# Crocodoctopus/zkstark

Measured on AMD Instinct MI355X. Metric: field-elements/s through LDE+Merkle+FRI (full STARK-101 prover), higher is better.
Workload: dtype u32 (mod 3*2^30+1) + SHA-256

## Files before the change

zkstark_amd/build.py:

```python
import concurrent.futures
import hashlib
import os
import shutil
import subprocess
import sys

HERE = os.path.dirname(os.path.abspath(__file__))
CSRC = os.path.join(HERE, "csrc")
OBJDIR = os.path.join(HERE, "build")
LIB = os.path.join(HERE, "libzkstark_amd.so")
HASHFILE = LIB + ".hash"
SOURCES = ["kernels.hip", "ntt_fast.hip", "domain.hip", "zkstark.hip", "batch.hip", "shard.hip", "verify.hip", "grind.hip", "host_sha.cpp", "version.cpp"]
HEADERS = ["field.hpp", "sha256.hpp", "blake2s.hpp", "sha256_quad.hpp", "fieldhash.hpp", "fieldhash_f64.hpp", "kernels.hpp", "transcript.hpp", "host_sha.hpp", "internal.hpp", "pool.hpp",
           "shard.hpp", "board.hpp", "peer.hpp", os.path.join("..", "..", "include", "zkstark_amd.h")]
ARCH = "gfx950"
FLAGS = ["-O3", "-std=c++17", f"--offload-arch={ARCH}", "-fPIC", "-Wall", "-Wno-unused-function"]
FLAGS += os.environ.get("ZK_BUILD_DEFS", "").split()


def _read(rel):
    with open(os.path.join(CSRC, rel), "rb") as f:
        return f.read()


def source_hash():
    h = hashlib.sha256()
    for rel in SOURCES + HEADERS:
        h.update(os.path.basename(rel).encode() + b"\0")
        h.update(_read(rel))
        h.update(b"\0")
    h.update(" ".join(FLAGS).encode())
    return h.hexdigest()[:24]


def built_hash():
    if not os.path.exists(LIB):
        return None
    try:
        with open(HASHFILE) as f:
            side = f.read().strip()
        if side and os.path.getmtime(HASHFILE) >= os.path.getmtime(LIB):
            return side
    except OSError:
        pass
    try:
        with open(LIB, "rb") as f:
# ... 68 lines not shown
```

zkstark_amd/csrc/internal.hpp:

```cpp
#pragma once
#include <hip/hip_runtime.h>

#include <cstddef>
#include <cstring>
#include <string>
#include <vector>

#include "../../include/zkstark_amd.h"
#include "field.hpp"
#include "kernels.hpp"
#include "transcript.hpp"

struct zk_channel {
    zk::Channel ch;
};

namespace zk {
namespace impl {

int fail(int code, const char* fmt, ...);
const char* last_error();

#define HIPCHK(expr)                                                                          \
    do {                                                                                      \
// ... 8 lines not shown
template <> struct AbiMin<zk_shard_options>   { static constexpr uint32_t v = 48;   static constexpr const char* name = "zk_shard_options"; };
template <> struct AbiMin<zk_shard_stats>     { static constexpr uint32_t v = 112;  static constexpr const char* name = "zk_shard_stats"; };
template <> struct AbiMin<zk_shard_plan_info> { static constexpr uint32_t v = 200;  static constexpr const char* name = "zk_shard_plan_info"; };
template <> struct AbiMin<zk_chain_probe>     { static constexpr uint32_t v = 48;   static constexpr const char* name = "zk_chain_probe"; };
template <class T> inline size_t abi_bytes(const T* p, const char* who) {
    static_assert(sizeof(T) >= AbiMin<T>::v && offsetof(T, struct_size) == 0, "a struct of the C ABI shrank or lost its size field");
    const uint32_t n = p->struct_size;
    if (n < AbiMin<T>::v || n > (1u << 16) || (n > AbiMin<T>::v && n < sizeof(T))) {
        fail(ZK_ERR_INVALID, "%s: %s.struct_size is %u; the caller sets it to sizeof(%s) before the call (ZK_STRUCT_INIT): at least %u bytes "
                             "(ABI version 6), %zu in this library (ABI version %u) -- was the caller compiled against another zkstark_amd.h?",
             who, AbiMin<T>::name, n, AbiMin<T>::name, AbiMin<T>::v, sizeof(T), (unsigned)ZK_ABI_VERSION);
        return 0;
    }
    return n < sizeof(T) ? n : sizeof(T);
}
template <class T> inline int abi_put(T* out, const T& src, const char* who) {
    const size_t k = abi_bytes(out, who);
    if (!k) return ZK_ERR_INVALID;
    memcpy(reinterpret_cast<char*>(out) + sizeof(uint32_t), reinterpret_cast<const char*>(&src) + sizeof(uint32_t), k - sizeof(uint32_t));
    return ZK_OK;
}
template <class T> inline int abi_get(const T* in, T* local, const char* who) {
    const size_t k = abi_bytes(in, who);
    if (!k) return ZK_ERR_INVALID;
    memset(static_cast<void*>(local), 0, sizeof(T));
    memcpy(static_cast<void*>(local), in, k);
    local->struct_size = (uint32_t)sizeof(T);
    return ZK_OK;
}

constexpr uint32_t kMaxQueries = 64;
constexpr uint32_t kHostTopSingle = 8;
constexpr uint32_t kMaxHostLog = 10;
constexpr size_t kMailValsOff = kMailDigests + ((size_t)8 << kMaxHostLog);
constexpr size_t kMailWords = kMailValsOff + ((size_t)2 << kMaxHostLog);
constexpr uint32_t kMaxRadixLog = 8;

inline int check_proof_size(const char* who, uint32_t log_n, uint32_t log_b, uint32_t log_extra = 0) {
    if (log_n < 2 || log_b < 1 || log_b > 5 || log_n + log_b + log_extra > 30)
        return fail(ZK_ERR_INVALID, "%s: need 2 <= log_n, 1 <= log_blowup <= 5, log_n + log_blowup%s <= 30 (got %u, %u)", who,
                    log_extra ? " + log_batch" : "", log_n, log_b);
    if (log_n == 3)
        return fail(ZK_ERR_INVALID, "%s: n = 8 is degenerate for the Fibonacci-square constraints (the degree asserts of prover.rs:156/:169 would fail)", who);
    return ZK_OK;
}

struct Plan {
    uint32_t nd = 0;
    uint32_t bits[kMaxDigits] = {0};
};
Plan make_plan(uint32_t log_m);
uint32_t pick_logC(uint32_t log_total, uint32_t logR);

struct DevTable {
    uint32_t* lo = nullptr;
    uint32_t* hi = nullptr;
    uint32_t lo_bits = 0;
    PowTable view() const { return PowTable{lo, hi, lo_bits}; }
};
int build_table(uint32_t root, uint32_t log_order, DevTable* t);
void free_table(DevTable* t);

int run_dif(const uint32_t* src, uint32_t* data, uint32_t log_m, const Plan& pl, PowTable tw_inv, uint32_t L, uint32_t scale_mont,
            hipStream_t s, Profiler* prof = nullptr, uint32_t batch = 1, size_t src_stride = 0, size_t data_stride = 0);
int run_dit(uint32_t* data, uint32_t log_m, const Plan& pl, PowTable tw, uint32_t L, hipStream_t s);

constexpr uint32_t kGrindHostMaxBits = 10;
struct Grinder;
// ... 59 lines not shown
```

zkstark_amd/csrc/zkstark.hip:

```cpp
#include <hip/hip_runtime.h>

#include <algorithm>
#include <chrono>
#include <cstdarg>
#include <cstdio>
#include <cstdlib>
#include <cstring>
#include <atomic>
#include <condition_variable>
#include <functional>
#include <mutex>
#include <new>
#include <thread>
#include <string>
#include <vector>

#include "../../include/zkstark_amd.h"
#include "field.hpp"
#include "kernels.hpp"
#include "sha256.hpp"
#include "transcript.hpp"
#include "host_sha.hpp"
#include "internal.hpp"
#include "pool.hpp"

using namespace zk;
using namespace zk::impl;

struct zk_ctx {
    int device = 0;
    uint32_t log_n = 0, log_b = 0, L = 0;
    size_t n = 0, N = 0, B = 0;
    uint32_t R = 0;
    hipStream_t stream = nullptr;
    zk_dom* dom = nullptr;
    uint32_t* d_trace = nullptr;
    uint32_t* d_coef = nullptr;
    uint32_t* d_layers = nullptr;
    std::vector<size_t> layer_off, layer_len;
    uint32_t* d_trees = nullptr;
    std::vector<size_t> tree_off;
    uint64_t* d_gather_off = nullptr;
    uint32_t* d_gather_out = nullptr;
    uint64_t* h_gather_off = nullptr;
    uint32_t* h_gather_out = nullptr;
    uint64_t* dm_gather_off = nullptr;
    uint32_t* dm_gather_out = nullptr;
    const uint32_t* host_nodes[40] = {};
    size_t host_node_cnt[40] = {};
    const uint32_t* host_vals[40] = {};
    std::vector<const uint32_t*> fetch_vals, fetch_nodes;
    std::vector<uint32_t> fetch_vdev;
    std::vector<uint64_t> fetch_ditems;
    std::vector<uint8_t> commit_buf;
    bool pending_top = false;
    uint32_t pending_tree = 0;
    size_t open_nv = 0, open_ndg = 0, open_vi = 0;
    bool open_pending = false;
    uint32_t* h_small = nullptr;
    uint32_t* h_mailbox = nullptr;
    uint32_t* d_mailbox = nullptr;
    uint32_t* d_counter = nullptr;
    bool counters_dirty = false;
    uint32_t mail_seq = 0;
    uint32_t tree_seq[40] = {};
    bool early = false, early_ok = false, gate_pending = false;
    uint32_t* h_gate = nullptr;
    uint32_t* d_gate = nullptr;
    uint32_t* h_dyn = nullptr;
    uint32_t* d_dyn = nullptr;
    uint32_t gate_seq = 0;
    uint32_t host_top = 0, host_tail = 0;
    Pool* pool = nullptr;
    uint32_t* h_stage = nullptr;
    uint32_t* d_stage = nullptr;
    size_t stage_words = 0, stage_used = 0;
    ScatterSeg* h_segs = nullptr;
    ScatterSeg* d_segs = nullptr;
    uint32_t n_segs = 0;
    double seg_words = 0;
    std::vector<uint32_t> tail_vals;
    uint32_t tail_log = 0;
    bool tail_have = false;
    double t_wait = 0, t_host_hash = 0, t_launch = 0;
    bool tail = false;
    uint32_t hinv_host = 0;
    uint32_t queries = 1;
    uint32_t grind = 0;
    Grinder* grinder = nullptr;
    uint32_t fold = 1;
    uint64_t skipped_layers = 0, skipped_trees = 0;
    bool coset = false;
    uint8_t tree_steps[40] = {};
    uint32_t stop = 0;
    uint32_t* d_final = nullptr;
    std::vector<uint32_t> final_poly;
    int hash = 0;
    bool checks = false;
    uint32_t* d_check = nullptr;
    DevTable ones;
    size_t gather_cap = 0;
    size_t device_bytes = 0;
    double setup_ms = 0;
    bool have_trace = false, have_lde = false;
    uint32_t first = 0, last = 0;
    zk_transcript_info info{};
    Profiler prof;
    zk_kernel_stat kstat[K_COUNT] = {};
};

namespace {

template <typename T>
int dmalloc(zk_ctx* c, T** p, size_t bytes) {
// ... 75 lines not shown
    if (rc) return rc;
    HIPCHK(launch_compose_merkle(a, c->d_trees + c->tree_off[1], c->stream, prof_of(c), mail_of(c, 1, true), c->hash));
    return ZK_OK;
}
int do_fold_commit(zk_ctx* c, uint32_t round, uint32_t beta_raw) {
    FoldArgs a;
    int rc = fold_args(c->dom, c->d_layers + c->layer_off[1 + round], c->d_layers + c->layer_off[2 + round], c->L - round, round, beta_raw, a);
    if (rc) return rc;
    HIPCHK(launch_fold_merkle(a, c->d_trees + c->tree_off[2 + round], c->stream, prof_of(c), mail_of(c, 2 + round, true), c->hash));
    return ZK_OK;
}

int wait_mail(zk_ctx* c, uint32_t seq) {
    double t0 = now_us();
    int rc = wait_flag(c->h_mailbox, seq, c->stream);
    c->t_wait += now_us() - t0;
    if (rc) c->counters_dirty = true;
    return rc;
}

int read_root(zk_ctx* c, uint32_t tree, uint8_t out[32]) {
    int rc = wait_mail(c, c->tree_seq[tree]);
    if (rc) return rc;
    digest_words_to_bytes(c->h_mailbox + kMailDigests, out);
    return ZK_OK;
}

uint32_t* stage_alloc(zk_ctx* c, size_t words) {
    if (c->stage_used + words > c->stage_words) return nullptr;
    uint32_t* p = c->h_stage + c->stage_used;
    c->stage_used += (words + 7) & ~(size_t)7;
    return p;
}
int stage_seg(zk_ctx* c, const uint32_t* src, size_t dst, size_t words, uint32_t kind) {
    if (c->n_segs >= 4 * 34) return fail(ZK_ERR_STATE, "scatter segment table full");
    c->h_segs[c->n_segs++] = ScatterSeg{(uint64_t)(src - c->h_stage), (uint64_t)dst, (uint32_t)words, kind};
    c->seg_words += (double)words;
    return ZK_OK;
}

int read_commit(zk_ctx* c, uint32_t tree, uint8_t root[32]) {
    const uint32_t H = top_of(c, tree);
    if (!H) return read_root(c, tree, root);
    const size_t cnt = (size_t)1 << H;
    uint32_t* nodes = stage_alloc(c, (2 * cnt - 1) * 8);
    if (!nodes) return fail(ZK_ERR_STATE, "host staging buffer exhausted");
    int rc = wait_mail(c, c->tree_seq[tree]);
    if (rc) return rc;
    double t0 = now_us();
    memcpy(nodes + 8 * (cnt - 1), c->h_mailbox + kMailDigests, cnt * 32);
    const uint32_t sub_log = host_sub_log();
    if (H > sub_log && c->pool) {
        const uint32_t top = H - sub_log;
        c->pool->run((size_t)1 << top, 1, [&](size_t sub) { host_sha_reduce_sub(nodes, H, top, sub); });
        host_sha_reduce(nodes, top);
    } else {
        host_sha_reduce(nodes, H);
    }
    digest_words_to_bytes(nodes, root);
    c->t_host_hash += now_us() - t0;
    if (c->tail_have && c->tail_log == layer_log(c, tree) && tree >= 1) {
        c->tail_vals.assign(c->h_mailbox + kMailValsOff, c->h_mailbox + kMailValsOff + ((size_t)1 << c->tail_log));
    }
    c->host_nodes[tree] = nodes;
    c->host_node_cnt[tree] = 2 * cnt - 1;
    return stage_seg(c, nodes, c->tree_off[tree], (cnt - 1) * 8, 0);
}

int host_fold_commit(zk_ctx* c, uint32_t round, uint32_t beta_raw, uint8_t root[32]) {
    const uint32_t log_out = c->L - round - 1;
    const size_t half = (size_t)1 << log_out;
    const double t_begin = now_us();
    uint32_t* vals = stage_alloc(c, half);
    uint32_t* nodes = stage_alloc(c, (2 * half - 1) * 8);
    if (!vals || !nodes) return fail(ZK_ERR_STATE, "host staging buffer exhausted");
    const zk_dom* d = c->dom;
    const uint32_t cc_m = to_mont(mulmod(beta_raw % P, d->fold_k[round]));
    const uint32_t step_m = to_mont(powmod(c->hinv_host, (uint64_t)1 << round));
    const uint32_t* in = c->tail_vals.data();
    uint32_t xinv_m = to_mont(1);
    for (size_t i = 0; i < half; ++i) {
        uint32_t u = in[i], v = in[i + half];
        vals[i] = add(mont_mul(add(u, v), d->inv2_mont), mont_mul(mont_mul(sub(u, v), xinv_m), cc_m));
        xinv_m = mont_mul(xinv_m, step_m);
    }
    host_sha_leaves(vals, half, nodes + 8 * (half - 1));
    host_sha_reduce(nodes, log_out);
    digest_words_to_bytes(nodes, root);
    c->tail_vals.assign(vals, vals + half);
    c->tail_log = log_out;
    c->t_host_hash += now_us() - t_begin;
    c->tree_steps[2 + round] = 0;
    c->host_vals[2 + round] = vals;
    c->host_nodes[2 + round] = nodes;
    c->host_node_cnt[2 + round] = 2 * half - 1;
    int rc = stage_seg(c, vals, c->layer_off[2 + round], half, 1);
    if (!rc) rc = stage_seg(c, nodes, c->tree_off[2 + round], (2 * half - 1) * 8, 0);
    return rc;
}

int fri_round_commit(zk_ctx* c, uint32_t round, uint32_t beta_raw, uint8_t root[32]) {
    if (c->tail_have && c->tail_log == c->L - round && c->L - round - 1 <= c->host_tail) return host_fold_commit(c, round, beta_raw, root);
    int rc = do_fold_commit(c, round, beta_raw);
    return rc ? rc : read_commit(c, 2 + round, root);
}
bool round_on_host(const zk_ctx* c, uint32_t round) {
    return c->hash == 0 && c->host_top && c->host_tail && c->L >= c->host_tail + 1 && c->L - round <= c->host_tail + 1;
}
bool can_gate(const zk_ctx* c, uint32_t round) { return c->fold == 1 && !c->coset && !c->stop && c->early && c->early_ok && !c->checks && round < c->R && !round_on_host(c, round); }
int enqueue_gated_fold(zk_ctx* c, uint32_t round) {
    FoldArgs a;
    int rc = fold_args(c->dom, c->d_layers + c->layer_off[1 + round], c->d_layers + c->layer_off[2 + round], c->L - round, round, 0u, a);
    if (rc) return rc;
    ++c->gate_seq;
    a.dyn = c->d_dyn + 16 * (c->gate_seq & 1u);
    HIPCHK(hipStreamWaitValue32(c->stream, c->d_gate, c->gate_seq, hipStreamWaitValueEq, 0xFFFFFFFFu));
    c->gate_pending = true;
    HIPCHK(launch_fold_merkle(a, c->d_trees + c->tree_off[2 + round], c->stream, prof_of(c), mail_of(c, 2 + round, true), c->hash));
    return ZK_OK;
}
void release_gate(zk_ctx* c, uint32_t c_mont) {
    c->h_dyn[16 * (c->gate_seq & 1u)] = c_mont;
    __atomic_store_n(c->h_gate, c->gate_seq, __ATOMIC_RELEASE);
    c->gate_pending = false;
}
void release_gated_fold(zk_ctx* c, uint32_t round, uint32_t beta_raw) {
    release_gate(c, to_mont(mulmod(beta_raw % P, c->dom->fold_k[round])));
}
struct GateGuard {
    zk_ctx* c;
    ~GateGuard() { if (c->gate_pending) release_gate(c, 0u); }
};

void begin_proof(zk_ctx* c) {
    c->stage_used = 0; c->n_segs = 0; c->seg_words = 0; c->tail_log = 0; c->tail_have = false;
    c->t_wait = c->t_host_hash = c->t_launch = 0;
    memset(c->host_nodes, 0, sizeof c->host_nodes);
    memset(c->host_node_cnt, 0, sizeof c->host_node_cnt);
    memset(c->host_vals, 0, sizeof c->host_vals);
}
int flush_host_parts(zk_ctx* c) {
    HIPCHK(launch_scatter(c->d_stage, c->d_segs, c->n_segs, c->seg_words, c->d_trees, c->d_layers, c->stream, prof_of(c)));
    c->n_segs = 0;
    c->pending_top = false;
    return ZK_OK;
}
int settle_pending(zk_ctx* c) { return c->pending_top ? flush_host_parts(c) : (int)ZK_OK; }
int last_layer_value(zk_ctx* c, uint32_t* out) {
    const uint32_t* v;
    if (c->tail_have && c->tail_log == c->log_b) v = c->tail_vals.data();
    else {
        HIPCHK(hipMemcpyAsync(c->h_small, c->d_layers + c->layer_off[1 + c->R], c->B * 4, hipMemcpyDeviceToHost, c->stream));
        HIPCHK(hipStreamSynchronize(c->stream));
        v = c->h_small;
    }
    for (size_t i = 1; i < c->B; ++i)
        if (v[i] != v[0]) return fail(ZK_ERR_CHECK, "last FRI layer is not constant (prover.rs:238): trace does not satisfy the constraints");
    *out = v[0];
    return ZK_OK;
}

int final_alloc(zk_ctx* c) {
    return c->d_final ? (int)ZK_OK : dmalloc(c, &c->d_final, (((size_t)1 << kFinalPolyMaxLog) + 1) * 4);
}
int final_poly_value(zk_ctx* c) {
    const uint32_t Rp = c->R - c->stop;
    const size_t cnt = (size_t)1 << c->stop;
    int rc = final_alloc(c);
    if (rc) return rc;
    if ((rc = dom_final_poly(c->dom, c->d_layers + c->layer_off[1 + Rp], c->d_final, c->L - Rp, Rp, (uint32_t)cnt, c->stream, prof_of(c)))) return rc;
    HIPCHK(hipMemcpyAsync(c->h_small, c->d_final, (cnt + 1) * 4, hipMemcpyDeviceToHost, c->stream));
    HIPCHK(hipStreamSynchronize(c->stream));
    if (c->h_small[0])
        return fail(ZK_ERR_CHECK, "final FRI layer has degree >= 2^%u: trace does not satisfy the constraints (%u non-zero coefficients above; cf. prover.rs:238)", c->stop, c->h_small[0]);
    c->final_poly.assign(c->h_small + 1, c->h_small + 1 + cnt);
    return ZK_OK;
}

int do_compose(zk_ctx* c, const uint32_t alpha_raw[3]) {
    return dom_compose(c->dom, c->d_layers + c->layer_off[0], c->d_layers + c->layer_off[1], c->first, c->last,
                       alpha_raw, c->stream, prof_of(c));
}

// ... 4 lines not shown


int checks_alloc(zk_ctx* c) {
    if (c->d_check) return ZK_OK;
    int rc = dmalloc(c, &c->d_check, (c->N + 2) * 4);
    if (rc) return rc;
    return build_table(1, c->log_n, &c->ones);
}
int check_interpolant(zk_ctx* c) {
    const zk_dom* d = c->dom;
    CoefPrepArgs pa{};
    pa.log_n = d->log_n; pa.log_b = d->log_b;
    pa.tw = d->H.view(); pa.wtab = c->ones.view(); pa.ninv_mont = d->ninv_mont;
    pa.nd = d->plan.nd;
    for (uint32_t t = 0; t < d->plan.nd; ++t) pa.dig_bits[t] = d->plan.bits[t];
    HIPCHK(launch_coef_prepare(c->d_coef, c->d_check, pa, c->stream));
    int rc = run_dit(c->d_check, d->log_n, d->plan, d->H.view(), d->L, c->stream);
    if (rc) return rc;
    std::vector<uint32_t> got(c->n), want(c->n);
    HIPCHK(hipMemcpyAsync(got.data(), c->d_check, c->n * 4, hipMemcpyDeviceToHost, c->stream));
    HIPCHK(hipMemcpyAsync(want.data(), c->d_trace, c->n * 4, hipMemcpyDeviceToHost, c->stream));
    HIPCHK(hipStreamSynchronize(c->stream));
    for (size_t i = 0; i + 1 < c->n; ++i)
        if (got[i] != want[i])
            return fail(ZK_ERR_CHECK, "self-check prover.rs:64-66 failed: f(g^%zu) = %u, trace value %u", i, got[i], want[i]);
    return ZK_OK;
}
int check_degree(zk_ctx* c, uint32_t layer, uint32_t want_deg, const char* cite) {
    const uint32_t lg = layer_log(c, layer);
    const size_t m = (size_t)1 << lg;
    const uint32_t* src = c->d_layers + c->layer_off[layer];
    if (lg <= 10) {
        std::vector<uint32_t> v(m);
        if (c->tail_have && c->tail_log == lg && layer >= 2) v.assign(c->tail_vals.begin(), c->tail_vals.begin() + m);
        else {
            HIPCHK(hipMemcpyAsync(v.data(), src, m * 4, hipMemcpyDeviceToHost, c->stream));
            HIPCHK(hipStreamSynchronize(c->stream));
        }
        const uint32_t winv = invmod(root_of_unity(lg));
        for (size_t k = m; k-- > want_deg; ) {
            uint32_t acc = 0, step = powmod(winv, k), x = 1;
            for (size_t i = 0; i < m; ++i) { acc = add(acc, mulmod(v[i], x)); x = mulmod(x, step); }
            if (k > want_deg && acc != 0)
                return fail(ZK_ERR_CHECK, "self-check %s failed: layer %u has a non-zero coefficient of degree %zu > %u", cite, layer, k, want_deg);
            if (k == want_deg && acc == 0)
                return fail(ZK_ERR_CHECK, "self-check %s failed: layer %u has degree below %u", cite, layer, want_deg);
        }
        return ZK_OK;
    }
    const Plan pl = make_plan(lg);
    int rc = run_dif(src, c->d_check, lg, pl, c->dom->Hinv.view(), c->dom->L, 0, c->stream);
    if (rc) return rc;
    uint32_t* res = c->d_check + c->N;
    HIPCHK(hipMemsetAsync(res, 0, 8, c->stream));
    HIPCHK(launch_degree_check(c->d_check, lg, pl.nd, pl.bits, want_deg + 1, res, c->stream));
    uint32_t h[2];
    HIPCHK(hipMemcpyAsync(h, res, 8, hipMemcpyDeviceToHost, c->stream));
    HIPCHK(hipStreamSynchronize(c->stream));
    if (h[0]) return fail(ZK_ERR_CHECK, "self-check %s failed: layer %u has %u non-zero coefficients of degree > %u (a division left a remainder)", cite, layer, h[0], want_deg);
    if (!h[1]) return fail(ZK_ERR_CHECK, "self-check %s failed: layer %u has degree below %u", cite, layer, want_deg);
    return ZK_OK;
}

void open_begin(zk_ctx* c, size_t nvals) {
    c->fetch_vals.assign(nvals, nullptr); c->fetch_vdev.assign(nvals, 0); c->fetch_nodes.clear(); c->fetch_ditems.clear();
    c->open_nv = c->open_ndg = c->open_vi = 0;
}
void open_val(zk_ctx* c, uint32_t layer, size_t x) {
    if (c->host_vals[layer]) c->fetch_vals[c->open_vi++] = c->host_vals[layer] + x;
    else { c->fetch_vdev[c->open_vi++] = (uint32_t)c->open_nv; c->h_gather_off[c->open_nv++] = (uint64_t)c->layer_off[layer] + x; }
}
void open_path(zk_ctx* c, uint32_t tree, size_t m, size_t leaf) {
    for (size_t i = leaf + m - 1; i != 0; i = (i - 1) >> 1) {
        const size_t nd = (i & 1) ? i + 1 : i - 1;
        if (nd < c->host_node_cnt[tree]) c->fetch_nodes.push_back(c->host_nodes[tree] + 8 * nd);
        else { c->fetch_nodes.push_back(c->h_gather_out + 8 * c->open_ndg); ++c->open_ndg; c->fetch_ditems.push_back((uint64_t)c->tree_off[tree] + (uint64_t)nd * 8); }
    }
}
int open_launch(zk_ctx* c) {
    const size_t nv = c->open_nv, ndg = c->open_ndg;
    if (nv + ndg > c->gather_cap) return fail(ZK_ERR_STATE, "gather capacity exceeded");
    if (ndg) memcpy(c->h_gather_off + nv, c->fetch_ditems.data(), ndg * 8);
    for (size_t i = 0; i < c->fetch_vals.size(); ++i)
        if (!c->fetch_vals[i]) c->fetch_vals[i] = c->h_gather_out + 8 * ndg + c->fetch_vdev[i];
    c->open_pending = nv + ndg != 0;
// ... 113 lines not shown
int prove_resident(zk_ctx* c, Channel& ch) {
    if (!c->have_trace) return fail(ZK_ERR_STATE, "zk_prove_resident: no trace uploaded");
    static const bool timing = getenv("ZK_HOST_TIMING") != nullptr;
    HostLaps lap{timing};
    const uint32_t R = c->R;
    ch.data.reserve(ch.data.size() + proof_data_len(c->log_n, c->log_b, c->queries, c->grind, c->fold, c->coset, c->stop));
    c->skipped_layers = c->skipped_trees = 0;
    uint8_t root[32];
    int rc;
    memset(&c->info, 0, sizeof c->info);
    c->info.public_last = c->last;
    c->pending_top = false;
    begin_proof(c);
    GateGuard gate_guard{c};
    if ((rc = do_lde(c))) return rc;
    if (c->checks && ((rc = checks_alloc(c)) || (rc = check_interpolant(c)))) return rc;
    if ((rc = do_merkle(c, 0, true))) return rc;
    if ((rc = read_commit(c, 0, root))) return rc;
    ch.commit_hash(root);
    memcpy(c->info.roots[0], root, 32);
    uint32_t alpha[3];
    for (int i = 0; i < 3; ++i) alpha[i] = c->info.alpha_raw[i] = ch.get_u32();
    if (c->coset) {
        if ((rc = do_compose(c, alpha)) || (rc = do_merkle(c, 1, true, false, fold_steps(R - c->stop, c->fold, 0)))) return rc;
    } else if ((rc = do_compose_commit(c, alpha))) return rc;
    if (can_gate(c, 0) && (rc = enqueue_gated_fold(c, 0))) return rc;
    if ((rc = read_commit(c, 1, root))) return rc;
    if (c->checks && (rc = check_degree(c, 1, (uint32_t)c->n - 1, "prover.rs:148-159/:169 (exact divisions, deg cp = n - 1)"))) return rc;
    ch.commit_hash(root);
    memcpy(c->info.roots[1], root, 32);
    if (c->fold > 1 || c->coset || c->stop) {
        if ((rc = prove_fold_rounds(c, ch))) return rc;
    } else for (uint32_t r = 0; r < R; ++r) {
        uint32_t beta = c->info.beta_raw[r] = ch.get_u32();
        if (c->gate_pending) {
            release_gated_fold(c, r, beta);
            if (can_gate(c, r + 1) && (rc = enqueue_gated_fold(c, r + 1))) return rc;
            if ((rc = read_commit(c, 2 + r, root))) return rc;
        } else if (c->tail_have && c->tail_log == c->L - r && c->L - r - 1 <= c->host_tail) {
            if ((rc = host_fold_commit(c, r, beta, root))) return rc;
        } else {
            if ((rc = do_fold_commit(c, r, beta))) return rc;
            if (can_gate(c, r + 1) && (rc = enqueue_gated_fold(c, r + 1))) return rc;
            if ((rc = read_commit(c, 2 + r, root))) return rc;
        }
        if (c->checks && (rc = check_degree(c, 2 + r, (uint32_t)(c->n >> (r + 1)) - ((c->n >> (r + 1)) ? 1 : 0), "prover.rs:228-251 (FRI layer degree)"))) return rc;
        ch.commit_hash(root);
        memcpy(c->info.roots[2 + r], root, 32);
    }
    lap("lde .. last root");
    if (timing) fprintf(stderr, "[zk timing]   of which: waiting for the device %.1f us, host hashing (tops + tail) %.1f us\n", c->t_wait, c->t_host_hash);
    return prove_finish(c, ch, lap);
}

}

namespace zk {
namespace impl {
int tail_open_begin(zk_ctx* c, size_t x) {
    if (!c || !c->tail) return fail(ZK_ERR_INVALID, "tail_open_begin: not a tail context");
    HIPCHK(hipSetDevice(c->device));
    open_begin(c, 2 * (size_t)c->R);
    for (uint32_t i = 0; i < c->R; ++i) {
        const size_t len = c->N >> i, xi = x % len, nx = (xi + len / 2) % len;
        open_val(c, 1 + i, xi); open_path(c, 1 + i, len, xi);
        open_val(c, 1 + i, nx); open_path(c, 1 + i, len, nx);
    }
    return open_launch(c);
}
int tail_open_end(zk_ctx* c, uint32_t* vals_out, uint8_t* paths_out) {
    int rc = open_wait(c);
    if (rc) return rc;
    for (size_t i = 0; i < c->fetch_vals.size(); ++i) vals_out[i] = *c->fetch_vals[i];
    for (size_t i = 0; i < c->fetch_nodes.size(); ++i) digest_words_to_bytes(c->fetch_nodes[i], paths_out + 32 * i);
    return ZK_OK;
}
int merkle_nodes_to_host(int device, hipStream_t s, const uint32_t* d_heap, size_t first, size_t count, uint8_t* out) {
    if (!count) return ZK_OK;
    HIPCHK(hipSetDevice(device));
    HIPCHK(hipMemcpyAsync(out, d_heap + first * 8, count * 32, hipMemcpyDeviceToHost, s));
    HIPCHK(hipStreamSynchronize(s));
// ... 34 lines not shown
    return mulmod(a % P, invmod(b % P));
}
uint32_t zk_field_rem(uint32_t a, uint32_t rhs) {
    if (rhs == 0) { fail(ZK_ERR_INVALID, "zk_field_rem: remainder by zero (field.rs:89-94 panics)"); return 0; }
    return (a % P) % rhs;
}
uint32_t zk_field_generator(void) {
    static const uint32_t g = [] {
        uint32_t factors[32], nf = 0, p = P - 1;
        for (uint32_t it = 2; p != 1; ++it) {
            if (p % it == 0) factors[nf++] = it;
            while (p % it == 0) p /= it;
        }
        for (uint32_t x = 2; x < P; ++x) {
            bool primitive = true;
            for (uint32_t i = 0; i < nf && primitive; ++i) primitive = powmod(x, (P - 1) / factors[i]) != 1;
            if (primitive) return x;
        }
        return 0u;
    }();
    return g;
}
uint32_t zk_field_order(uint32_t a) {
    a %= P;
    if (a == 0) return 0;
    uint32_t ord = P - 1;
    if (powmod(a, ord / 3) == 1) ord /= 3;
    while (ord % 2 == 0 && powmod(a, ord / 2) == 1) ord /= 2;
    return ord;
}
uint32_t zk_field_root_of_unity(uint32_t log_order) { return log_order > 30 ? 0 : root_of_unity(log_order); }

static int ctx_make(int device, uint32_t log_n, uint32_t log_b, uint32_t shift, bool tail, zk_ctx** out);
static int ctx_team(zk_ctx* c) {
    const uint32_t sub_log = host_sub_log();
    const unsigned want = c->host_top > sub_log ? (1u << (c->host_top - sub_log)) - 1u : 0u;
    if (c->pool && c->pool->workers() == want) return ZK_OK;
    delete c->pool;
    c->pool = nullptr;
    if (!want) return ZK_OK;
    const double spin_us = 5000.0;
    c->pool = new (std::nothrow) Pool(want, spin_us);
    return c->pool ? (int)ZK_OK : fail(ZK_ERR_NOMEM, "out of host memory");
}

int zk_ctx_create(int device, uint32_t log_n, uint32_t log_b, zk_ctx** out) {
    if (!out) return fail(ZK_ERR_INVALID, "zk_ctx_create: out is null");
    *out = nullptr;
    if (int rc = check_proof_size("zk_ctx_create", log_n, log_b)) return rc;
    return ctx_make(device, log_n, log_b, GEN_W, false, out);
}

static int ctx_make(int device, uint32_t log_n, uint32_t log_b, uint32_t shift, bool tail, zk_ctx** out) {
    auto t0 = std::chrono::steady_clock::now();
    HIPCHK(hipSetDevice(device));
    zk_ctx* c = new (std::nothrow) zk_ctx();
    if (!c) return fail(ZK_ERR_NOMEM, "out of host memory");
    c->device = device;
    c->log_n = log_n; c->log_b = log_b; c->L = log_n + log_b;
    c->n = (size_t)1 << log_n; c->B = (size_t)1 << log_b; c->N = c->n << log_b;
    c->R = log_n;
    int rc = ZK_OK;
    auto bail = [&](int code) { zk_ctx_destroy(c); return code; };
#define HIPCHK_C(expr)                                                                        \
    do {                                                                                      \
        hipError_t _e = (expr);                                                               \
        if (_e != hipSuccess) {                                                               \
            zk_ctx_destroy(c);                                                                \
            return fail(ZK_ERR_HIP, "%s failed: %s (%s:%d)", #expr, hipGetErrorString(_e), __FILE__, __LINE__); \
// ... 16 lines not shown
        c->tree_off.push_back(off);
        off += (2 * layer_size(c, l) - 1) * 8;
    }
    size_t tree_words = off;
    if ((rc = dmalloc(c, &c->d_trace, c->n * 4))) return bail(rc);
    if ((rc = dmalloc(c, &c->d_coef, 2 * c->n * 4))) return bail(rc);
    if ((rc = dmalloc(c, &c->d_layers, layer_words * 4))) return bail(rc);
    if ((rc = dmalloc(c, &c->d_trees, tree_words * 4))) return bail(rc);
    c->gather_cap = (size_t)kMaxQueries * (4 + 2 * c->R) * (c->L + 1) + 64;
    if ((rc = dmalloc(c, &c->d_gather_off, c->gather_cap * 8))) return bail(rc);
    if ((rc = dmalloc(c, &c->d_gather_out, c->gather_cap * 32))) return bail(rc);
    HIPCHK_C(hipHostMalloc((void**)&c->h_gather_off, c->gather_cap * 8, hipHostMallocMapped | hipHostMallocCoherent));
    HIPCHK_C(hipHostMalloc((void**)&c->h_gather_out, c->gather_cap * 32, hipHostMallocMapped | hipHostMallocCoherent));
    HIPCHK_C(hipHostGetDevicePointer((void**)&c->dm_gather_off, c->h_gather_off, 0));
    HIPCHK_C(hipHostGetDevicePointer((void**)&c->dm_gather_out, c->h_gather_out, 0));
    HIPCHK_C(hipHostMalloc((void**)&c->h_small, 4096));
    const size_t mail_bytes = kMailWords * 4;
    if ((rc = dmalloc(c, &c->d_counter, 64))) return bail(rc);
    HIPCHK_C(hipMemsetAsync(c->d_counter, 0, 64, c->stream));
    HIPCHK_C(hipHostMalloc((void**)&c->h_mailbox, mail_bytes, hipHostMallocMapped | hipHostMallocCoherent));
    memset(c->h_mailbox, 0, mail_bytes);
    HIPCHK_C(hipHostGetDevicePointer((void**)&c->d_mailbox, c->h_mailbox, 0));
    HIPCHK_C(hipHostMalloc((void**)&c->h_gate, 64, hipHostMallocMapped | hipHostMallocCoherent));
    HIPCHK_C(hipHostMalloc((void**)&c->h_dyn, 2 * 16 * 4, hipHostMallocMapped | hipHostMallocCoherent));
    memset(c->h_gate, 0, 64);
    memset(c->h_dyn, 0, 2 * 16 * 4);
    HIPCHK_C(hipHostGetDevicePointer((void**)&c->d_gate, c->h_gate, 0));
    HIPCHK_C(hipHostGetDevicePointer((void**)&c->d_dyn, c->h_dyn, 0));
    {
        int can = 0;
        if (hipDeviceGetAttribute(&can, hipDeviceAttributeCanUseStreamWaitValue, device) != hipSuccess) { can = 0; (void)hipGetLastError(); }
        c->early_ok = can != 0 && !tail;
    }
    c->stage_words = (size_t)(c->R + 2) * ((size_t)16 << kMaxHostLog) + ((size_t)64 << kMaxHostLog);
    const size_t seg_bytes = 4 * 34 * sizeof(ScatterSeg);
    HIPCHK_C(hipHostMalloc((void**)&c->h_stage, c->stage_words * 4 + seg_bytes, hipHostMallocMapped | hipHostMallocCoherent));
    HIPCHK_C(hipHostGetDevicePointer((void**)&c->d_stage, c->h_stage, 0));
    c->h_segs = reinterpret_cast<ScatterSeg*>(c->h_stage + c->stage_words);
    c->d_segs = reinterpret_cast<ScatterSeg*>(c->d_stage + c->stage_words);
    if (host_sha_available()) {
        c->host_top = 8;
        c->host_tail = 9;
    }
    if (int prc = ctx_team(c)) { zk_ctx_destroy(c); return prc; }
#undef HIPCHK_C
    c->setup_ms = std::chrono::duration<double, std::milli>(std::chrono::steady_clock::now() - t0).count();
    *out = c;
    return ZK_OK;
}

#ifdef ZK_WG_TRACE
extern "C++" { namespace zk { void dump_wg_trace(); } }
#endif

int zk_ctx_destroy(zk_ctx* c) {
    if (!c) return ZK_OK;
    (void)hipSetDevice(c->device);
    if (c->stream) (void)hipStreamSynchronize(c->stream);
#ifdef ZK_WG_TRACE
    zk::dump_wg_trace();
#endif
    dom_free(c->dom);
    if (c->d_trace) (void)hipFree(c->d_trace);
    if (c->d_coef) (void)hipFree(c->d_coef);
    if (c->d_layers) (void)hipFree(c->d_layers);
    if (c->d_trees) (void)hipFree(c->d_trees);
    if (c->d_counter) (void)hipFree(c->d_counter);
    if (c->d_check) (void)hipFree(c->d_check);
// ... 92 lines not shown
    }
    c->stop = stop_log;
    return ZK_OK;
}
uint32_t zk_ctx_get_fri_stop(const zk_ctx* c) { return c ? c->stop : 0; }
int zk_ctx_final_poly(const zk_ctx* c, uint32_t* out, size_t cap, size_t* count) {
    if (!c || !count || (!out && cap)) return fail(ZK_ERR_INVALID, "zk_ctx_final_poly: null argument");
    if (c->final_poly.empty()) return fail(ZK_ERR_STATE, "zk_ctx_final_poly: no proof made yet");
    *count = c->final_poly.size();
    if (c->final_poly.size() > cap) return fail(ZK_ERR_BUFFER, "zk_ctx_final_poly: %zu coefficients, room for %zu", c->final_poly.size(), cap);
    memcpy(out, c->final_poly.data(), c->final_poly.size() * 4);
    return ZK_OK;
}
int zk_ctx_set_queries(zk_ctx* c, uint32_t n_queries) {
    if (!c) return fail(ZK_ERR_INVALID, "null context");
    if (n_queries < 1 || n_queries > kMaxQueries) return fail(ZK_ERR_INVALID, "zk_ctx_set_queries: need 1 <= n_queries <= %u", kMaxQueries);
    c->queries = n_queries;
    return ZK_OK;
}
int zk_ctx_set_grinding(zk_ctx* c, uint32_t grind_bits) {
    if (!c) return fail(ZK_ERR_INVALID, "null context");
    if (c->tail) return fail(ZK_ERR_STATE, "zk_ctx_set_grinding: FRI-tail context");
    if (grind_bits > kMaxGrindBits) return fail(ZK_ERR_INVALID, "zk_ctx_set_grinding: need grind_bits <= %u (got %u)", kMaxGrindBits, grind_bits);
    if (grind_bits > kGrindHostMaxBits && !c->grinder) {
        HIPCHK(hipSetDevice(c->device));
        if (int rc = grinder_create(c->device, c->stream, 1, &c->grinder)) return rc;
    }
    c->grind = grind_bits;
    return ZK_OK;
}

int zk_ctx_set_host_levels(zk_ctx* c, uint32_t top_log, uint32_t tail_log) {
    if (!c) return fail(ZK_ERR_INVALID, "null context");
    if (top_log > kMaxHostLog || tail_log > kMaxHostLog || (tail_log && !top_log))
        return fail(ZK_ERR_INVALID, "zk_ctx_set_host_levels: need top_log, tail_log <= %u, and top_log > 0 when tail_log > 0", kMaxHostLog);
    c->host_top = top_log;
    c->host_tail = tail_log;
    return ctx_team(c);
}
int zk_ctx_get_host_levels(const zk_ctx* c, uint32_t* top_log, uint32_t* tail_log) {
    if (!c || !top_log || !tail_log) return fail(ZK_ERR_INVALID, "zk_ctx_get_host_levels: null argument");
    *top_log = c->host_top;
    *tail_log = c->host_tail;
    return ZK_OK;
}
int zk_ctx_set_checks(zk_ctx* c, int on) {
    if (!c) return fail(ZK_ERR_INVALID, "null context");
    if (c->tail) return fail(ZK_ERR_STATE, "zk_ctx_set_checks: FRI-tail context");
    c->checks = on != 0;
    return ZK_OK;
}
static const char kNoBlake2s[] = "BLAKE2s (hash 2) is not built for this entry point yet";
int zk_ctx_set_hash(zk_ctx* c, int hash_kind) {
    if (!c) return fail(ZK_ERR_INVALID, "null context");
    if (hash_kind != ZK_HASH_SHA256 && hash_kind != ZK_HASH_FIELD && hash_kind != ZK_HASH_BLAKE2S)
        return fail(ZK_ERR_INVALID, "zk_ctx_set_hash: unknown hash %d", hash_kind);
    if (hash_kind == ZK_HASH_BLAKE2S && c->tail) return fail(ZK_ERR_INVALID, "zk_ctx_set_hash: %s", kNoBlake2s);
    c->hash = hash_kind;
    return ZK_OK;
}

int zk_ctx_set_profiling(zk_ctx* c, uint32_t class_mask) {
    if (!c) return fail(ZK_ERR_INVALID, "null context");
    c->prof.mask = class_mask & ((1u << K_COUNT) - 1u);
    return ZK_OK;
}

static int put_kernel_stats(zk_kernel_stat* out, size_t count, const zk_kernel_stat* src, const char* who) {
// ... 894 lines not shown
```

Before: 2.937 billion.

## Parallelize host FRI tail folding and hashing across a thread pool

Moves the host-side FRI tail fold plus SHA-256 leaf/tree hashing into a chunked, pool-parallel routine and allows host tail layers up to 2^13. Tail values are now referenced in place instead of being copied into a vector each round, and scatter segments are split into bounded pieces. The pool size is capped by the usable CPU cores and cgroup quota. Larger host tails require a bigger pinned staging buffer and mailbox, and the parallel path is only used when the tail level is raised.

```diff
diff --git a/zkstark_amd/build.py b/zkstark_amd/build.py
--- a/zkstark_amd/build.py
+++ b/zkstark_amd/build.py
@@ -11,7 +11,7 @@
 LIB = os.path.join(HERE, "libzkstark_amd.so")
 HASHFILE = LIB + ".hash"
 SOURCES = ["kernels.hip", "ntt_fast.hip", "domain.hip", "zkstark.hip", "batch.hip", "shard.hip", "verify.hip", "grind.hip", "host_sha.cpp", "version.cpp"]
-HEADERS = ["field.hpp", "sha256.hpp", "blake2s.hpp", "sha256_quad.hpp", "fieldhash.hpp", "fieldhash_f64.hpp", "kernels.hpp", "transcript.hpp", "host_sha.hpp", "internal.hpp", "pool.hpp",
+HEADERS = ["field.hpp", "sha256.hpp", "blake2s.hpp", "sha256_quad.hpp", "fieldhash.hpp", "fieldhash_f64.hpp", "kernels.hpp", "transcript.hpp", "host_sha.hpp", "host_tail.hpp", "internal.hpp", "pool.hpp",
            "shard.hpp", "board.hpp", "peer.hpp", os.path.join("..", "..", "include", "zkstark_amd.h")]
 ARCH = "gfx950"
 FLAGS = ["-O3", "-std=c++17", f"--offload-arch={ARCH}", "-fPIC", "-Wall", "-Wno-unused-function"]
diff --git a/zkstark_amd/csrc/host_tail.hpp b/zkstark_amd/csrc/host_tail.hpp
--- /dev/null
+++ b/zkstark_amd/csrc/host_tail.hpp
@@ -0,0 +1,74 @@
+#pragma once
+#include <stddef.h>
+#include <stdint.h>
+
+#include "field.hpp"
+#include "host_sha.hpp"
+#include "pool.hpp"
+
+#ifndef ZK_TAIL_CHUNK_LOG
+#define ZK_TAIL_CHUNK_LOG 7
+#endif
+#ifndef ZK_TAIL_TEAM_MIN_LOG
+#define ZK_TAIL_TEAM_MIN_LOG 10
+#endif
+#ifndef ZK_TAIL_TEAM_MAX
+#define ZK_TAIL_TEAM_MAX 7
+#endif
+
+namespace zk {
+
+constexpr uint32_t kTailChunkMinLog = 4;
+constexpr uint32_t kTailChunkLog = ZK_TAIL_CHUNK_LOG;
+constexpr uint32_t kTailTeamMinLog = ZK_TAIL_TEAM_MIN_LOG;
+constexpr uint32_t kTailTeamMax = ZK_TAIL_TEAM_MAX;
+static_assert(kTailChunkLog >= kTailChunkMinLog && kTailChunkLog <= 12, "host tail chunk size");
+static_assert(kTailTeamMinLog > kTailChunkLog && kTailTeamMinLog <= 13, "a team round has at least two chunks");
+static_assert(kTailTeamMax >= 1 && kTailTeamMax <= 15, "host tail team size");
+
+struct HostTailConsts {
+    uint32_t cc_m, step_m;
+};
+inline HostTailConsts host_tail_consts(uint32_t beta_raw, uint32_t fold_k, uint32_t step) {
+    return HostTailConsts{to_mont(mulmod(beta_raw % P, fold_k)), to_mont(step)};
+}
+
+inline void host_tail_fold(const uint32_t* in, size_t half, size_t start, size_t count, uint32_t xinv_m, HostTailConsts k, uint32_t inv2_m,
+                           uint32_t* vals) {
+    for (size_t i = start; i < start + count; ++i) {
+        const uint32_t u = in[i], v = in[i + half];
+        vals[i] = add(mont_mul(add(u, v), inv2_m), mont_mul(mont_mul(sub(u, v), xinv_m), k.cc_m));
+        xinv_m = mont_mul(xinv_m, k.step_m);
+    }
+}
+
+inline void host_tail_round_serial(const uint32_t* in, uint32_t log_out, HostTailConsts k, uint32_t inv2_m, uint32_t* vals, uint32_t* nodes) {
+    const size_t half = (size_t)1 << log_out;
+    host_tail_fold(in, half, 0, half, to_mont(1), k, inv2_m, vals);
+    host_sha_leaves(vals, half, nodes + 8 * (half - 1));
+    host_sha_reduce(nodes, log_out);
+}
+
+inline bool host_tail_uses_team(const Pool* pool, uint32_t log_out, uint32_t chunk_log = kTailChunkLog, uint32_t team_min_log = kTailTeamMinLog) {
+    return pool && pool->workers() && log_out >= team_min_log && log_out > chunk_log && chunk_log >= kTailChunkMinLog;
+}
+
+inline void host_tail_round(const uint32_t* in, uint32_t log_out, HostTailConsts k, uint32_t inv2_m, Pool* pool, uint32_t* vals, uint32_t* nodes,
+                            uint32_t chunk_log = kTailChunkLog, uint32_t team_min_log = kTailTeamMinLog) {
+    if (!host_tail_uses_team(pool, log_out, chunk_log, team_min_log)) {
+        host_tail_round_serial(in, log_out, k, inv2_m, vals, nodes);
+        return;
+    }
+    const size_t half = (size_t)1 << log_out, chunk = (size_t)1 << chunk_log;
+    const uint32_t top = log_out - chunk_log;
+    const uint32_t step = mont_mul(k.step_m, 1u);
+    pool->run((size_t)1 << top, 1, [&](size_t c) {
+        const size_t start = c * chunk;
+        host_tail_fold(in, half, start, chunk, to_mont(powmod(step, start)), k, inv2_m, vals);
+        host_sha_leaves(vals + start, chunk, nodes + 8 * (half - 1 + start));
+        host_sha_reduce_sub(nodes, log_out, top, c);
+    });
+    host_sha_reduce(nodes, top);
+}
+
+}
diff --git a/zkstark_amd/csrc/internal.hpp b/zkstark_amd/csrc/internal.hpp
--- a/zkstark_amd/csrc/internal.hpp
+++ b/zkstark_amd/csrc/internal.hpp
@@ -64,8 +64,9 @@
 constexpr uint32_t kMaxQueries = 64;
 constexpr uint32_t kHostTopSingle = 8;
 constexpr uint32_t kMaxHostLog = 10;
+constexpr uint32_t kMaxHostTailLog = 13;
 constexpr size_t kMailValsOff = kMailDigests + ((size_t)8 << kMaxHostLog);
-constexpr size_t kMailWords = kMailValsOff + ((size_t)2 << kMaxHostLog);
+constexpr size_t kMailWords = kMailValsOff + ((size_t)2 << kMaxHostTailLog);
 constexpr uint32_t kMaxRadixLog = 8;
 
 inline int check_proof_size(const char* who, uint32_t log_n, uint32_t log_b, uint32_t log_extra = 0) {
diff --git a/zkstark_amd/csrc/zkstark.hip b/zkstark_amd/csrc/zkstark.hip
--- a/zkstark_amd/csrc/zkstark.hip
+++ b/zkstark_amd/csrc/zkstark.hip
@@ -1,4 +1,5 @@
 #include <hip/hip_runtime.h>
+#include <sched.h>
 
 #include <algorithm>
 #include <chrono>
@@ -23,6 +24,7 @@
 #include "host_sha.hpp"
 #include "internal.hpp"
 #include "pool.hpp"
+#include "host_tail.hpp"
 
 using namespace zk;
 using namespace zk::impl;
@@ -79,7 +81,7 @@
     ScatterSeg* d_segs = nullptr;
     uint32_t n_segs = 0;
     double seg_words = 0;
-    std::vector<uint32_t> tail_vals;
+    const uint32_t* tail_vals = nullptr;
     uint32_t tail_log = 0;
     bool tail_have = false;
     double t_wait = 0, t_host_hash = 0, t_launch = 0;
@@ -221,9 +223,14 @@
     c->stage_used += (words + 7) & ~(size_t)7;
     return p;
 }
+constexpr size_t kSegPieceWords = (size_t)1 << 13;
+constexpr uint32_t kMaxSegs = 256;
 int stage_seg(zk_ctx* c, const uint32_t* src, size_t dst, size_t words, uint32_t kind) {
-    if (c->n_segs >= 4 * 34) return fail(ZK_ERR_STATE, "scatter segment table full");
-    c->h_segs[c->n_segs++] = ScatterSeg{(uint64_t)(src - c->h_stage), (uint64_t)dst, (uint32_t)words, kind};
+    for (size_t at = 0; at < words; at += kSegPieceWords) {
+        const size_t n = words - at < kSegPieceWords ? words - at : kSegPieceWords;
+        if (c->n_segs >= kMaxSegs) return fail(ZK_ERR_STATE, "scatter segment table full");
+        c->h_segs[c->n_segs++] = ScatterSeg{(uint64_t)(src - c->h_stage) + at, (uint64_t)dst + at, (uint32_t)n, kind};
+    }
     c->seg_words += (double)words;
     return ZK_OK;
 }
@@ -234,6 +241,9 @@
     const size_t cnt = (size_t)1 << H;
     uint32_t* nodes = stage_alloc(c, (2 * cnt - 1) * 8);
     if (!nodes) return fail(ZK_ERR_STATE, "host staging buffer exhausted");
+    if (c->pool && c->host_tail >= kTailTeamMinLog && c->fold == 1 && !c->coset && !c->stop && tree >= 1 && c->L >= c->host_tail + 1 &&
+        layer_log(c, tree) > c->host_tail && layer_log(c, tree) <= c->host_tail + 3)
+        c->pool->run(c->pool->workers() + 1, 1, [](size_t) {});
     int rc = wait_mail(c, c->tree_seq[tree]);
     if (rc) return rc;
     double t0 = now_us();
@@ -249,7 +259,7 @@
     digest_words_to_bytes(nodes, root);
     c->t_host_hash += now_us() - t0;
     if (c->tail_have && c->tail_log == layer_log(c, tree) && tree >= 1) {
-        c->tail_vals.assign(c->h_mailbox + kMailValsOff, c->h_mailbox + kMailValsOff + ((size_t)1 << c->tail_log));
+        c->tail_vals = c->h_mailbox + kMailValsOff;
     }
     c->host_nodes[tree] = nodes;
     c->host_node_cnt[tree] = 2 * cnt - 1;
@@ -264,19 +274,10 @@
     uint32_t* nodes = stage_alloc(c, (2 * half - 1) * 8);
     if (!vals || !nodes) return fail(ZK_ERR_STATE, "host staging buffer exhausted");
     const zk_dom* d = c->dom;
-    const uint32_t cc_m = to_mont(mulmod(beta_raw % P, d->fold_k[round]));
-    const uint32_t step_m = to_mont(powmod(c->hinv_host, (uint64_t)1 << round));
-    const uint32_t* in = c->tail_vals.data();
-    uint32_t xinv_m = to_mont(1);
-    for (size_t i = 0; i < half; ++i) {
-        uint32_t u = in[i], v = in[i + half];
-        vals[i] = add(mont_mul(add(u, v), d->inv2_mont), mont_mul(mont_mul(sub(u, v), xinv_m), cc_m));
-        xinv_m = mont_mul(xinv_m, step_m);
-    }
-    host_sha_leaves(vals, half, nodes + 8 * (half - 1));
-    host_sha_reduce(nodes, log_out);
+    const HostTailConsts k = host_tail_consts(beta_raw, d->fold_k[round], powmod(c->hinv_host, (uint64_t)1 << round));
+    host_tail_round(c->tail_vals, log_out, k, d->inv2_mont, c->pool, vals, nodes);
     digest_words_to_bytes(nodes, root);
-    c->tail_vals.assign(vals, vals + half);
+    c->tail_vals = vals;
     c->tail_log = log_out;
     c->t_host_hash += now_us() - t_begin;
     c->tree_steps[2 + round] = 0;
@@ -322,7 +323,7 @@
 };
 
 void begin_proof(zk_ctx* c) {
-    c->stage_used = 0; c->n_segs = 0; c->seg_words = 0; c->tail_log = 0; c->tail_have = false;
+    c->stage_used = 0; c->n_segs = 0; c->seg_words = 0; c->tail_log = 0; c->tail_have = false; c->tail_vals = nullptr;
     c->t_wait = c->t_host_hash = c->t_launch = 0;
     memset(c->host_nodes, 0, sizeof c->host_nodes);
     memset(c->host_node_cnt, 0, sizeof c->host_node_cnt);
@@ -337,7 +338,7 @@
 int settle_pending(zk_ctx* c) { return c->pending_top ? flush_host_parts(c) : (int)ZK_OK; }
 int last_layer_value(zk_ctx* c, uint32_t* out) {
     const uint32_t* v;
-    if (c->tail_have && c->tail_log == c->log_b) v = c->tail_vals.data();
+    if (c->tail_have && c->tail_log == c->log_b) v = c->tail_vals;
     else {
         HIPCHK(hipMemcpyAsync(c->h_small, c->d_layers + c->layer_off[1 + c->R], c->B * 4, hipMemcpyDeviceToHost, c->stream));
         HIPCHK(hipStreamSynchronize(c->stream));
@@ -408,7 +409,7 @@
     const uint32_t* src = c->d_layers + c->layer_off[layer];
     if (lg <= 10) {
         std::vector<uint32_t> v(m);
-        if (c->tail_have && c->tail_log == lg && layer >= 2) v.assign(c->tail_vals.begin(), c->tail_vals.begin() + m);
+        if (c->tail_have && c->tail_log == lg && layer >= 2) v.assign(c->tail_vals, c->tail_vals + m);
         else {
             HIPCHK(hipMemcpyAsync(v.data(), src, m * 4, hipMemcpyDeviceToHost, c->stream));
             HIPCHK(hipStreamSynchronize(c->stream));
@@ -425,8 +426,9 @@
         return ZK_OK;
     }
     const Plan pl = make_plan(lg);
-    int rc = run_dif(src, c->d_check, lg, pl, c->dom->Hinv.view(), c->dom->L, 0, c->stream);
-    if (rc) return rc;
+    int rc;
+    if (c->host_vals[layer] && (rc = flush_host_parts(c))) return rc;
+    if ((rc = run_dif(src, c->d_check, lg, pl, c->dom->Hinv.view(), c->dom->L, 0, c->stream))) return rc;
     uint32_t* res = c->d_check + c->N;
     HIPCHK(hipMemsetAsync(res, 0, 8, c->stream));
     HIPCHK(launch_degree_check(c->d_check, lg, pl.nd, pl.bits, want_deg + 1, res, c->stream));
@@ -606,6 +608,8 @@
     if (c->fold > 1 || c->coset || c->stop) {
         if ((rc = prove_fold_rounds(c, ch))) return rc;
     } else for (uint32_t r = 0; r < R; ++r) {
+        const double t_round = timing ? now_us() : 0.0;
+        bool on_host = false;
         uint32_t beta = c->info.beta_raw[r] = ch.get_u32();
         if (c->gate_pending) {
             release_gated_fold(c, r, beta);
@@ -613,6 +617,7 @@
             if ((rc = read_commit(c, 2 + r, root))) return rc;
         } else if (c->tail_have && c->tail_log == c->L - r && c->L - r - 1 <= c->host_tail) {
             if ((rc = host_fold_commit(c, r, beta, root))) return rc;
+            on_host = true;
         } else {
             if ((rc = do_fold_commit(c, r, beta))) return rc;
             if (can_gate(c, r + 1) && (rc = enqueue_gated_fold(c, r + 1))) return rc;
@@ -621,6 +626,8 @@
         if (c->checks && (rc = check_degree(c, 2 + r, (uint32_t)(c->n >> (r + 1)) - ((c->n >> (r + 1)) ? 1 : 0), "prover.rs:228-251 (FRI layer degree)"))) return rc;
         ch.commit_hash(root);
         memcpy(c->info.roots[2 + r], root, 32);
+        if (timing)
+            fprintf(stderr, "[zk timing]   round %2u -> 2^%-2u values, %s %7.1f us\n", r, c->L - r - 1, on_host ? "host  " : "device", now_us() - t_round);
     }
     lap("lde .. last root");
     if (timing) fprintf(stderr, "[zk timing]   of which: waiting for the device %.1f us, host hashing (tops + tail) %.1f us\n", c->t_wait, c->t_host_hash);
@@ -721,9 +728,28 @@
 uint32_t zk_field_root_of_unity(uint32_t log_order) { return log_order > 30 ? 0 : root_of_unity(log_order); }
 
 static int ctx_make(int device, uint32_t log_n, uint32_t log_b, uint32_t shift, bool tail, zk_ctx** out);
+static unsigned usable_cores() {
+    unsigned n = 1;
+    cpu_set_t set;
+    CPU_ZERO(&set);
+    if (sched_getaffinity(0, sizeof set, &set) == 0 && CPU_COUNT(&set) > 0) n = (unsigned)CPU_COUNT(&set);
+    if (FILE* f = fopen("/sys/fs/cgroup/cpu.max", "r")) {
+        char q[32] = {0};
+        long long period = 0;
+        if (fscanf(f, "%31s %lld", q, &period) == 2 && strcmp(q, "max") != 0 && period > 0) {
+            const long long quota = (atoll(q) + period - 1) / period;
+            if (quota >= 1 && (unsigned long long)quota < n) n = (unsigned)quota;
+        }
+        fclose(f);
+    }
+    return n;
+}
 static int ctx_team(zk_ctx* c) {
     const uint32_t sub_log = host_sub_log();
-    const unsigned want = c->host_top > sub_log ? (1u << (c->host_top - sub_log)) - 1u : 0u;
+    const unsigned top_want = c->host_top > sub_log ? (1u << (c->host_top - sub_log)) - 1u : 0u;
+    const unsigned tail_want = c->host_tail >= kTailTeamMinLog ? std::min((1u << (c->host_tail - kTailChunkLog)) - 1u, kTailTeamMax) : 0u;
+    const unsigned cores = usable_cores();
+    const unsigned want = std::min({std::max(top_want, tail_want), 15u, cores - 1u});
     if (c->pool && c->pool->workers() == want) return ZK_OK;
     delete c->pool;
     c->pool = nullptr;
@@ -806,8 +832,8 @@
         if (hipDeviceGetAttribute(&can, hipDeviceAttributeCanUseStreamWaitValue, device) != hipSuccess) { can = 0; (void)hipGetLastError(); }
         c->early_ok = can != 0 && !tail;
     }
-    c->stage_words = (size_t)(c->R + 2) * ((size_t)16 << kMaxHostLog) + ((size_t)64 << kMaxHostLog);
-    const size_t seg_bytes = 4 * 34 * sizeof(ScatterSeg);
+    c->stage_words = (size_t)(c->R + 2) * ((size_t)16 << kMaxHostLog) + ((size_t)40 << kMaxHostTailLog);
+    const size_t seg_bytes = kMaxSegs * sizeof(ScatterSeg);
     HIPCHK_C(hipHostMalloc((void**)&c->h_stage, c->stage_words * 4 + seg_bytes, hipHostMallocMapped | hipHostMallocCoherent));
     HIPCHK_C(hipHostGetDevicePointer((void**)&c->d_stage, c->h_stage, 0));
     c->h_segs = reinterpret_cast<ScatterSeg*>(c->h_stage + c->stage_words);
@@ -966,8 +992,9 @@
 
 int zk_ctx_set_host_levels(zk_ctx* c, uint32_t top_log, uint32_t tail_log) {
     if (!c) return fail(ZK_ERR_INVALID, "null context");
-    if (top_log > kMaxHostLog || tail_log > kMaxHostLog || (tail_log && !top_log))
-        return fail(ZK_ERR_INVALID, "zk_ctx_set_host_levels: need top_log, tail_log <= %u, and top_log > 0 when tail_log > 0", kMaxHostLog);
+    if (top_log > kMaxHostLog || tail_log > kMaxHostTailLog || (tail_log && !top_log) || (tail_log > kMaxHostLog && top_log < kHostTopSingle))
+        return fail(ZK_ERR_INVALID, "zk_ctx_set_host_levels: need top_log <= %u, tail_log <= %u, top_log > 0 when tail_log > 0 and top_log >= %u when tail_log > %u",
+                    kMaxHostLog, kMaxHostTailLog, kHostTopSingle, kMaxHostLog);
     c->host_top = top_log;
     c->host_tail = tail_log;
     return ctx_team(c);
```

After: 2.935 billion. No clear change (-0.1%).
